# Exidekat/TransformerUpscaler

Measured on AMD Instinct MI355X. Metric: images/sec, FastTransformer 2x 720p->1080p inference, higher is better.
Workload: dtype bf16

## Files before the change

### transformerupscaler_amd/csrc/conv12_fused.hip

```cpp
#include "conv_pingpong.h"

namespace {

constexpr int TH = 8, TW = 32, HALO_W = TW + 2, HALO_H = TH + 2, NPIX_HALO = HALO_H * HALO_W;
constexpr int IN_BYTES = NPIX_HALO * 128;
constexpr int WROWS = 64, WSLAB = WROWS * 128;
constexpr int NRUNS = (NPIX_HALO + 15) / 16;
constexpr int RUNS_PER_WAVE = (NRUNS + 3) / 4;
constexpr size_t C12_LDS = (size_t)9 * WSLAB + 2 * (size_t)IN_BYTES + 256 + 256 + 256;
static_assert(C12_LDS <= 163840, "LDS budget");

__global__ __launch_bounds__(256) void conv1_compact_kernel(const float* __restrict__ x, u32x2* __restrict__ xc, int H, int W,
                                                            int Hp, int Wp)
{
    const int xp = blockIdx.y * 256 + threadIdx.x;
    if (xp >= Wp) return;
    const int row = blockIdx.x, b = row / Hp, yp = row - b * Hp;
    const int iy = yp - 2, ix = xp - 2;
    float v0 = 0.f, v1 = 0.f, v2 = 0.f;
    if (iy >= 0 && iy < H && ix >= 0 && ix < W) {
        const size_t plane = (size_t)H * W;
        const float* s = x + (size_t)b * 3 * plane + (size_t)iy * W + ix;
        v0 = s[0]; v1 = s[plane]; v2 = s[2 * plane];
    }
    xc[(size_t)row * Wp + xp] = u32x2{pack_bf16x2(v0, v1), pack_bf16x2(v2, 0.f)};
}

__global__ __launch_bounds__(512, 2) void conv12_fused_kernel(
    const bf16_t* __restrict__ xc, const bf16_t* __restrict__ w1, const float* __restrict__ b1,
    const bf16_t* __restrict__ wp, const float* __restrict__ bias, bf16_t* __restrict__ out,
    int B, int H, int W, int Wp, int img_bytes, int tilesX, int tilesY)
{
    extern __shared__ __attribute__((aligned(16))) char smem[];
    char* w_lds = smem;
    char* in_lds = smem + 9 * WSLAB;

    const int grp = __builtin_amdgcn_readfirstlane((int)(threadIdx.x >> 8));
    const int tid = threadIdx.x & 255, lane = tid & 63, wave = tid >> 6;
    const int wave_u = __builtin_amdgcn_readfirstlane(wave);
    const int g = lane >> 4, p = lane & 15;
    const int total_tiles = tilesX * tilesY * B;
    char* my_in = in_lds + grp * IN_BYTES;
    float* bias_lds = reinterpret_cast<float*>(in_lds + 2 * IN_BYTES);
    uint32_t* tab_lds = reinterpret_cast<uint32_t*>(in_lds + 2 * IN_BYTES + 512);

    uint32_t poff[9][2];
    pixel_frag_offsets<3, HALO_W>(poff, my_in, wave, g, p);
    const uint32_t wbase0 = weight_frag_base(w_lds, g, p);

    f32x4 acc[4][4];
    const uint32_t bias_addr = lds_addr(bias_lds) + (uint32_t)(g * 64);

    auto store_tile = [&](const TC& c) {
#pragma unroll
        for (int pg = 0; pg < 4; ++pg) {
            const int oy = c.ty * TH + 2 * wave + (pg >> 1);
            const int ox = c.tx * TW + (pg & 1) * 16 + p;
            const bool ok = oy < H && ox < W;
            const size_t eoff = (((size_t)c.b * H + oy) * W + ox) * 64 + g * 16;
            uint32_t pk[8];
#pragma unroll
            for (int ct = 0; ct < 4; ++ct) {
                pk[ct * 2 + 0] = relu_pack_bf16x2(acc[pg][ct][0], acc[pg][ct][1]);
                pk[ct * 2 + 1] = relu_pack_bf16x2(acc[pg][ct][2], acc[pg][ct][3]);
            }
            bf16_t* o = ok ? out + eoff : reinterpret_cast<bf16_t*>(tup_store_sink) + lane * 16;
            *reinterpret_cast<u32x4*>(o) = u32x4{pk[0], pk[1], pk[2], pk[3]};
            *reinterpret_cast<u32x4*>(o + 8) = u32x4{pk[4], pk[5], pk[6], pk[7]};
        }
    };

    struct Conv1In { uint32_t raw[RUNS_PER_WAVE][8]; bf16x8 a[4]; };
    auto issue_conv1_loads = [&](const TC& c, Conv1In& in) {
        const int l = lane_id_fresh(), lg = l >> 4, lp = l & 15;
        const bf16_t* wrow = w1 + lp * 32 + lg * 8;
#pragma unroll
        for (int ct = 0; ct < 4; ++ct) in.a[ct] = *reinterpret_cast<const bf16x8*>(wrow + ct * 512);
        const u32x4 so = *reinterpret_cast<const u32x4*>(tab_lds + lg * 16);
        const uint32_t so4 = tab_lds[lg * 16 + 4];
        const int cb = __builtin_amdgcn_readfirstlane(c.b), cty = __builtin_amdgcn_readfirstlane(c.ty);
        const int ctx = __builtin_amdgcn_readfirstlane(c.tx);
        const char* img = reinterpret_cast<const char*>(xc) + (size_t)cb * img_bytes;
        const __amdgpu_buffer_rsrc_t rs = __builtin_amdgcn_make_buffer_rsrc((void*)img, 0, img_bytes, 0x00020000);
        const int tbase = (cty * TH * Wp + ctx * TW) * 8;
#pragma unroll
        for (int j = 0; j < RUNS_PER_WAVE; ++j) {
            const int G = wave_u + 4 * j;
            const int q = min(16 * G + lp, NPIX_HALO - 1);
            const int hy = (q * 241) >> 13, hx = q - hy * HALO_W;
            const int pix = (hy * Wp + hx) * 8;
            uint32_t* r = in.raw[j];
            r[0] = __builtin_amdgcn_raw_buffer_load_b32(rs, pix + (int)so[0] + 4, tbase, 0);
            const u32x2 s1 = __builtin_amdgcn_raw_buffer_load_b64(rs, pix + (int)so[1], tbase, 0);
            const u32x2 s2 = __builtin_amdgcn_raw_buffer_load_b64(rs, pix + (int)so[2], tbase, 0);
            const u32x2 s3 = __builtin_amdgcn_raw_buffer_load_b64(rs, pix + (int)so[3], tbase, 0);
            r[7] = __builtin_amdgcn_raw_buffer_load_b32(rs, pix + (int)so4, tbase, 0);
            r[1] = s1[0]; r[2] = s1[1]; r[3] = s2[0]; r[4] = s2[1]; r[5] = s3[0]; r[6] = s3[1];
        }
    };
    auto build_conv1 = [&](const TC& c, const Conv1In& in) {
        const int l = lane_id_fresh(), lg = l >> 4, lp = l & 15;
        const u32x4 sel = *reinterpret_cast<const u32x4*>(tab_lds + lg * 16 + 8);
        f32x4 bv[4];
#pragma unroll
        for (int ct = 0; ct < 4; ++ct) bv[ct] = *reinterpret_cast<const f32x4*>(bias_lds + 64 + lg * 16 + ct * 4);
        const int ty0 = c.ty * TH, tx0 = c.tx * TW;
        const bool edge = !(ty0 >= 1 && ty0 + TH + 1 <= H && tx0 >= 1 && tx0 + TW + 1 <= W);
        const uint32_t img_lds = lds_addr(my_in);
#pragma unroll
        for (int j = 0; j < RUNS_PER_WAVE; ++j) {
            const int G = wave_u + 4 * j;
            const uint32_t* r = in.raw[j];
            const u32x4 bw = {__builtin_amdgcn_perm(r[1], r[0], sel[0]), __builtin_amdgcn_perm(r[3], r[2], sel[1]),
                              __builtin_amdgcn_perm(r[5], r[4], sel[2]), __builtin_amdgcn_perm(r[7], r[6], sel[3])};
            const bf16x8 bfrag = __builtin_bit_cast(bf16x8, bw);
            f32x4 a[4];
#pragma unroll
            for (int ct = 0; ct < 4; ++ct) a[ct] = mfma16x16x32(in.a[ct], bfrag, bv[ct]);
            uint32_t pk[8];
#pragma unroll
            for (int ct = 0; ct < 4; ++ct) {
                pk[ct * 2 + 0] = relu_pack_bf16x2(a[ct][0], a[ct][1]);
                pk[ct * 2 + 1] = relu_pack_bf16x2(a[ct][2], a[ct][3]);
            }
            const int q = 16 * G + lp;
            if (edge) {
                const int hy = (q * 241) >> 13, hx = q - hy * HALO_W;
                const bool ok = (unsigned)(ty0 - 1 + hy) < (unsigned)H && (unsigned)(tx0 - 1 + hx) < (unsigned)W;
#pragma unroll
                for (int k = 0; k < 8; ++k) pk[k] = ok ? pk[k] : 0u;
            }
            const uint32_t a0 = img_lds + (uint32_t)swz128(q, 2 * lg), a1 = a0 ^ 16u;
            if (q < NPIX_HALO) {
                *reinterpret_cast<__attribute__((address_space(3))) u32x4*>(a0) = u32x4{pk[0], pk[1], pk[2], pk[3]};
                *reinterpret_cast<__attribute__((address_space(3))) u32x4*>(a1) = u32x4{pk[4], pk[5], pk[6], pk[7]};
            }
            __builtin_amdgcn_sched_barrier(0);
        }
    };

    const TileWalk walk(total_tiles, tilesX, tilesY, grp, true);
    const int my_count = walk.my_count, nphases = walk.nphases;
    const TC c_first = walk.first;

    stage_weights<4, 9>(w_lds, wp);
    if (threadIdx.x < 128) bias_lds[threadIdx.x] = threadIdx.x < 64 ? bias[threadIdx.x] : b1[threadIdx.x - 64];
    if (threadIdx.x < 64) {
        constexpr uint32_t X = 0x05040100u, Y = 0x01000706u, Z = 0x07060504u, F = 0x03020100u, Zero = 0x0c0c0c0cu;
        constexpr int slot_dydx[4][5] = {{0x00, 0x00, 0x01, 0x01, 0x02}, {0x02, 0x10, 0x10, 0x11, 0x12},
                                         {0x12, 0x12, 0x20, 0x21, 0x21}, {0x22, 0x22, 0x22, 0x22, 0x22}};
        constexpr uint32_t sels[4][4] = {{Z, X, Y, Z}, {X, Y, Z, X}, {Y, Z, X, Y}, {Z, F, Zero, Zero}};
        const int gg = threadIdx.x >> 4, w = threadIdx.x & 15;
        uint32_t v = 0u;
        if (w < 5) v = (uint32_t)((((slot_dydx[gg][w] >> 4) * Wp) + (slot_dydx[gg][w] & 15)) * 8);
        else if (w >= 8 && w < 12) v = sels[gg][w - 8];
        tab_lds[threadIdx.x] = v;
    }
    __syncthreads();
    if (grp == 0 && my_count > 0) {
        Conv1In in;
        issue_conv1_loads(c_first, in);
        build_conv1(c_first, in);
    }
    asm volatile("s_waitcnt lgkmcnt(0)" ::: "memory");
    __syncthreads();
    TC c_done = c_first, c_next = c_first;
    if (grp == 0) walk.advance(c_next);

    for (int ph = 0; ph < nphases; ++ph) {
        const int k = ph >> 1;
        if ((ph & 1) == grp) {
            if (k < my_count) k_loop<4, 9>(acc, poff, wbase0, bias_addr);
        } else {
            const int done = grp == 0 ? k : k - 1;
            const int nxt = done + 1;
            const bool store = done >= 0 && done < my_count;
            const bool fetch = nxt < my_count;
            if (fetch && store) {
                Conv1In in;
                issue_conv1_loads(c_next, in);
                __builtin_amdgcn_sched_barrier(0);
                store_tile(c_done);
                __builtin_amdgcn_sched_barrier(0);
                build_conv1(c_next, in);
            } else if (fetch) {
                Conv1In in;
                issue_conv1_loads(c_next, in);
                build_conv1(c_next, in);
            } else if (store) {
                store_tile(c_done);
            }
            c_done = c_next;
            walk.advance(c_next);
        }
        asm volatile("s_waitcnt lgkmcnt(0)" ::: "memory");
        __builtin_amdgcn_s_barrier();
    }
    asm volatile("s_waitcnt vmcnt(0)" ::: "memory");
}

}

extern "C" int tup_conv1_compact_fwd(const float* x, void* xc, int B, int H, int W, void* stream)
{
    if (B <= 0 || H <= 0 || W <= 0) return 0;
    const int Hp = (H + TH - 1) / TH * TH + 4, Wp = (W + TW - 1) / TW * TW + 4;
    if ((long long)B * Hp > 0x7fffffffLL) return (int)hipErrorInvalidValue;
    conv1_compact_kernel<<<dim3((unsigned)(B * Hp), (unsigned)((Wp + 255) / 256)), dim3(256), 0, reinterpret_cast<hipStream_t>(stream)>>>(
        x, (u32x2*)xc, H, W, Hp, Wp);
    TUP_CHECK_LAUNCH();
    return 0;
}

extern "C" int tup_conv12_fused_fwd(const void* xc, const void* w1, const float* b1, const void* w2, const float* b2, void* out,
                                    int B, int H, int W, void* stream)
{
    if (B <= 0 || H <= 0 || W <= 0) return 0;
    const int tilesX = (W + TW - 1) / TW, tilesY = (H + TH - 1) / TH;
    const int Hp = tilesY * TH + 4, Wp = tilesX * TW + 4;
    const long long nt = (long long)tilesX * tilesY * B;
    if (nt > 0x7fffffffLL || (long long)Hp * Wp * 8 > 0x7fffffffLL) return (int)hipErrorInvalidValue;
    hipStream_t s = reinterpret_cast<hipStream_t>(stream);
    TUP_SET_DYN_LDS(conv12_fused_kernel, C12_LDS);
    const int grid = (int)(nt < 256 ? nt : 256);
    conv12_fused_kernel<<<dim3(grid), dim3(512), C12_LDS, s>>>((const bf16_t*)xc, (const bf16_t*)w1, b1, (const bf16_t*)w2, b2,
                                                               (bf16_t*)out, B, H, W, Wp, Hp * Wp * 8, tilesX, tilesY);
    TUP_CHECK_LAUNCH();
    return 0;
}
```

### transformerupscaler_amd/csrc/conv_pingpong.h

```cpp
#pragma once
#include "common.h"

namespace {

[[maybe_unused]] __device__ __attribute__((aligned(16))) unsigned int tup_zero_line[4] = {0u, 0u, 0u, 0u};
[[maybe_unused]] __device__ __attribute__((aligned(16))) unsigned int tup_store_sink[64 * 8];

#define TUP_ADD_DPP(acc, v, ctrl) asm("v_add_f32_dpp %0, %1, %0 " ctrl " row_mask:0xf bank_mask:0xf bound_ctrl:1" : "+v"(acc) : "v"(v))

TUP_DEVICE uint32_t relu_pack_bf16x2(float lo, float hi) {
    typedef short s16x2 __attribute__((ext_vector_type(2)));
    const bf16x2 v = __builtin_convertvector(f32x2{lo, hi}, bf16x2);
    return __builtin_bit_cast(uint32_t, __builtin_elementwise_max(__builtin_bit_cast(s16x2, v), s16x2{0, 0}));
}

TUP_DEVICE void xcd_band(int total, bool use_bands, int& first, int& stride, int& limit) {
    if ((gridDim.x & 7) == 0 && use_bands) {
        const int band = (total + 7) >> 3, start = (blockIdx.x & 7) * band;
        limit = min(total, start + band);
        first = start + (blockIdx.x >> 3);
        stride = gridDim.x >> 3;
    } else {
        limit = total; first = blockIdx.x; stride = gridDim.x;
    }
}

struct TC { int tx, ty, b; };

struct TileWalk {
    int my_count;
    int nphases;
    TC first;
    int tilesX, tilesY, step_x, step_y, step_b;

    TUP_DEVICE TileWalk(int total_tiles, int tilesX_, int tilesY_, int grp, bool use_bands) : tilesX(tilesX_), tilesY(tilesY_) {
        int first0, per, limit;
        xcd_band(total_tiles, use_bands, first0, per, limit);
        const int first_tile = first0 + grp * per, stride = 2 * per;
        my_count = first_tile < limit ? (limit - first_tile + stride - 1) / stride : 0;
        const int cnt0 = first0 < limit ? (limit - first0 + stride - 1) / stride : 0;
        nphases = 2 * cnt0 + 1;
        first.tx = first_tile % tilesX; const int t = first_tile / tilesX; first.ty = t % tilesY; first.b = t / tilesY;
        step_x = stride % tilesX; step_y = (stride / tilesX) % tilesY; step_b = stride / (tilesX * tilesY);
    }
    TUP_DEVICE void advance(TC& c) const {
        c.tx += step_x;
        if (c.tx >= tilesX) { c.tx -= tilesX; ++c.ty; }
        c.ty += step_y; c.b += step_b;
        if (c.ty >= tilesY) { c.ty -= tilesY; ++c.b; }
    }
};

template <int HALO_H, int HALO_W, int PAD>
struct HaloDma {
    static constexpr int IN_CHUNKS = HALO_H * HALO_W * 8, NPIECE = (IN_CHUNKS + 255) / 256;
    static constexpr bool LAST_PARTIAL = (IN_CHUNKS % 256) != 0;
    int rel[NPIECE];
    int tid, wave;
    bool last_ok;

    TUP_DEVICE HaloDma(int W, int tid_) : tid(tid_), wave(tid_ >> 6), last_ok((NPIECE - 1) * 256 + tid_ < IN_CHUNKS) {
#pragma unroll
        for (int it = 0; it < NPIECE; ++it) {
            const int idx = LAST_PARTIAL ? min(it * 256 + tid, IN_CHUNKS - 1) : it * 256 + tid;
            const int q = idx >> 3, c = (idx & 7) ^ ((q >> 1) & 7);
            const int yy = q / HALO_W, xx = q - yy * HALO_W;
            rel[it] = ((yy - PAD) * W + (xx - PAD)) * 128 + c * 16;
        }
    }
    TUP_DEVICE void prefetch(const bf16_t* x, int b, int ty0, int tx0, int H, int W, char* my_in, const void* zero) const {
        const char* xb = reinterpret_cast<const char*>(x + (size_t)b * H * W * 64);
        if (ty0 >= PAD && ty0 + HALO_H - PAD <= H && tx0 >= PAD && tx0 + HALO_W - PAD <= W) {
            const char* tb = xb + ((size_t)ty0 * W + tx0) * 128;
#pragma unroll
            for (int it = 0; it < NPIECE; ++it) {
                if (LAST_PARTIAL && it == NPIECE - 1 && !last_ok) continue;
                __builtin_amdgcn_global_load_lds((const __attribute__((address_space(1))) void*)(tb + rel[it]),
                                                 (__attribute__((address_space(3))) void*)(my_in + (it * 256 + wave * 64) * 16), 16, 0, 0);
            }
            return;
        }
#pragma unroll 1
        for (int base = 0; base < IN_CHUNKS; base += 256) {
            const int idx = base + tid;
            if (!LAST_PARTIAL || idx < IN_CHUNKS) {
                const int q = idx >> 3, cphys = idx & 7;
                const int c = cphys ^ ((q >> 1) & 7);
                const int yy = q / HALO_W, xx = q - yy * HALO_W;
                const int iy = ty0 - PAD + yy, ix = tx0 - PAD + xx;
                const void* src = (iy >= 0 && iy < H && ix >= 0 && ix < W)
                                      ? (const void*)(xb + ((size_t)(iy * W + ix) * 128 + c * 16)) : zero;
                __builtin_amdgcn_global_load_lds((const __attribute__((address_space(1))) void*)src,
                                                 (__attribute__((address_space(3))) void*)(my_in + (base + wave * 64) * 16), 16, 0, 0);
            }
        }
    }
};

template <int KS, int HALO_W>
TUP_DEVICE void pixel_frag_offsets(uint32_t (&poff)[KS * KS][2], const char* my_in, int wave, int g, int p) {
#pragma unroll
    for (int tap = 0; tap < KS * KS; ++tap)
#pragma unroll
        for (int rw = 0; rw < 2; ++rw)
            poff[tap][rw] = lds_addr(my_in) + (uint32_t)swz128((2 * wave + rw) * HALO_W + p + (tap / KS) * HALO_W + (tap % KS), g);
}
TUP_DEVICE uint32_t weight_frag_base(const char* w_lds, int g, int p) { return lds_addr(w_lds) + (uint32_t)swz128(p, g); }

template <int CT, int NTAPS>
TUP_DEVICE void k_loop(f32x4 (&acc)[4][CT], const uint32_t (&poff)[NTAPS][2], uint32_t wbase0, uint32_t bias_addr) {
    constexpr int WROWS = CT * 16;
    const uint32_t wbase1 = wbase0 ^ 64u;
    const uint32_t wbase0h = wbase0 + 57344u, wbase1h = wbase1 + 57344u;
#pragma unroll
    for (int ct = 0; ct < CT; ++ct) acc[0][ct] = __builtin_bit_cast(f32x4, lds_read_b128_asm(bias_addr + ct * 16));
    lds_wait<0>();
#pragma unroll
    for (int pg = 1; pg < 4; ++pg)
#pragma unroll
        for (int ct = 0; ct < CT; ++ct) acc[pg][ct] = acc[0][ct];
    constexpr int NSTEPS = NTAPS * 2;
    constexpr int PER = 4 + CT;
    constexpr int NM = 4 * CT;
    bf16x8 pf[3][4], wf[3][CT];
    auto load_one = [&](int step, int slot, int j) {
        const int tap = step >> 1;
        if (j < 4) {
            pf[slot][j] = (step & 1) ? lds_read_b128_asm_off_x64(poff[tap][j >> 1], (j & 1) * 2048)
                                     : lds_read_b128_asm_off(poff[tap][j >> 1], (j & 1) * 2048);
        } else {
            const int ct = j - 4;
            const int woff = (tap * WROWS + ct * 16) * 128;
            wf[slot][ct] = woff < 57344 ? lds_read_b128_asm_off((step & 1) ? wbase1 : wbase0, woff)
                                        : lds_read_b128_asm_off((step & 1) ? wbase1h : wbase0h, woff - 57344);
        }
    };
#pragma unroll
    for (int j = 0; j < PER; ++j) load_one(0, 0, j);
#pragma unroll
    for (int j = 0; j < PER; ++j) load_one(1, 1, j);
#pragma unroll
    for (int step = 0; step < NSTEPS; ++step) {
        const int cur = step % 3;
        if (step + 1 < NSTEPS) lds_wait<PER>(); else lds_wait<0>();
        __builtin_amdgcn_sched_barrier(0);
        int rd = 0;
#pragma unroll
        for (int m = 0; m < NM; ++m) {
            if (step + 2 < NSTEPS) {
#pragma unroll
                for (int j = 0; j < PER; ++j)
                    if (j == rd && j * NM < (m + 1) * PER) { load_one(step + 2, (step + 2) % 3, j); ++rd; }
            }
            const int pg = m / CT, ct = m % CT;
            acc[pg][ct] = mfma16x16x32(wf[cur][ct], pf[cur][pg], acc[pg][ct]);
            __builtin_amdgcn_sched_barrier(0);
        }
    }
}

template <int CT, int NTAPS>
TUP_DEVICE void stage_weights(char* w_lds, const bf16_t* wsrc) {
    for (int idx = threadIdx.x; idx < NTAPS * CT * 16 * 8; idx += 512) {
        const int row = idx >> 3, c = idx & 7;
        *reinterpret_cast<u32x4*>(w_lds + swz128(row, c)) = *reinterpret_cast<const u32x4*>(wsrc + (size_t)idx * 8);
    }
}
template <int CT, bool THIN>
TUP_DEVICE void stage_bias(float* bias_lds, const float* bias, int nt, int cout_valid) {
    if (threadIdx.x < 16 * CT) {
        const int gg = threadIdx.x / (4 * CT), ct = (threadIdx.x / 4) % CT, e = threadIdx.x & 3;
        float bval = 0.f;
        if (bias) {
            if constexpr (!THIN) bval = bias[nt * 64 + gg * 16 + ct * 4 + e];
            else { const int co = 16 * ct + 4 * gg + e; bval = co < cout_valid ? bias[co] : 0.f; }
        }
        bias_lds[threadIdx.x] = bval;
    }
}

}
```

### transformerupscaler_amd/csrc/decoder_fused.hip

```cpp
#include "conv_pingpong.h"

namespace {

constexpr int TH = 8, TW = 32, HALO_W = TW + 2, HALO_H = TH + 2, NPIX_HALO = HALO_H * HALO_W;
constexpr int IN_BYTES = NPIX_HALO * 128;
constexpr int WROWS = 64, WSLAB = WROWS * 128;
constexpr size_t DEC_LDS = (size_t)9 * WSLAB + 2 * (size_t)IN_BYTES + 256;
static_assert(DEC_LDS <= 163840, "LDS budget");

__global__ __launch_bounds__(512, 2) void decoder_fused_kernel(
    const bf16_t* __restrict__ x, const bf16_t* __restrict__ wp, const float* __restrict__ bias,
    const bf16_t* __restrict__ wz, float* __restrict__ part, float* __restrict__ seamv, float* __restrict__ cseam,
    int B, int H, int W, int tilesX, int tilesY)
{
    extern __shared__ __attribute__((aligned(16))) char smem[];
    char* w_lds = smem;
    char* in_lds = smem + 9 * WSLAB;

    const int grp = __builtin_amdgcn_readfirstlane((int)(threadIdx.x >> 8));
    const int tid = threadIdx.x & 255, lane = tid & 63, wave = tid >> 6;
    const int g = lane >> 4, p = lane & 15;
    const int total_tiles = tilesX * tilesY * B;
    char* my_in = in_lds + grp * IN_BYTES;

    using Dma = HaloDma<HALO_H, HALO_W, 1>;
    constexpr int NPIECE = Dma::NPIECE;
    const Dma dma(W, tid);
    auto prefetch_tile = [&](const TC& c) { dma.prefetch(x, c.b, c.ty * TH, c.tx * TW, H, W, my_in, tup_zero_line); };

    uint32_t poff[9][2];
    pixel_frag_offsets<3, HALO_W>(poff, my_in, wave, g, p);
    const uint32_t wbase0 = weight_frag_base(w_lds, g, p);

    f32x4 acc[4][4];
    float* bias_lds = reinterpret_cast<float*>(in_lds + 2 * IN_BYTES);
    const uint32_t bias_addr = lds_addr(bias_lds) + (uint32_t)(g * 64);
    bf16x8 zf[3][2];
    const uint32_t wz_voff = (uint32_t)(p * 128 + g * 16);
    auto load_zf = [&]() {
#pragma unroll
        for (int dy = 0; dy < 3; ++dy) {
            const bf16_t* base = wz + dy * 1024;
            asm volatile("global_load_dwordx4 %0, %1, %2" : "=v"(zf[dy][0]) : "v"(wz_voff), "s"(base));
            asm volatile("global_load_dwordx4 %0, %1, %2 offset:64" : "=v"(zf[dy][1]) : "v"(wz_voff), "s"(base));
        }
    };

    auto store_tile = [&](const TC& c) {
        const int b = c.b, y0 = c.ty * TH + 2 * wave, x0 = c.tx * TW;
        const bool edge = c.ty * TH + TH > H || x0 + TW > W;
        f32x4 z[4][3];
#pragma unroll
        for (int pg = 0; pg < 4; ++pg) {
            typedef short s16x2 __attribute__((ext_vector_type(2)));
            uint32_t pk[8];
#pragma unroll
            for (int ct = 0; ct < 4; ++ct) {
                pk[ct * 2 + 0] = pack_bf16x2(acc[pg][ct][0], acc[pg][ct][1]);
                pk[ct * 2 + 1] = pack_bf16x2(acc[pg][ct][2], acc[pg][ct][3]);
            }
#pragma unroll
            for (int q = 0; q < 8; ++q)
                pk[q] = __builtin_bit_cast(uint32_t, __builtin_elementwise_max(__builtin_bit_cast(s16x2, pk[q]), s16x2{0, 0}));
            if (edge) {
                const bool ok = y0 + (pg >> 1) < H && x0 + (pg & 1) * 16 + p < W;
#pragma unroll
                for (int q = 0; q < 8; ++q) pk[q] = ok ? pk[q] : 0u;
            }
            const bf16x8 b0 = __builtin_bit_cast(bf16x8, u32x4{pk[0], pk[1], pk[2], pk[3]});
            const bf16x8 b1 = __builtin_bit_cast(bf16x8, u32x4{pk[4], pk[5], pk[6], pk[7]});
#pragma unroll
            for (int dy = 0; dy < 3; ++dy) {
                z[pg][dy] = mfma16x16x32(zf[dy][0], b0, f32x4{0.f, 0.f, 0.f, 0.f});
                z[pg][dy] = mfma16x16x32(zf[dy][1], b1, z[pg][dy]);
            }
        }
        __builtin_amdgcn_sched_barrier(0);
        asm volatile("s_nop 7\n\ts_nop 7\n\ts_nop 4" ::: "memory");
        __builtin_amdgcn_sched_barrier(0);
        float h[2][2][3];
#pragma unroll
        for (int rw = 0; rw < 2; ++rw)
#pragma unroll
            for (int dy = 0; dy < 3; ++dy) {
                const f32x4 l = z[2 * rw][dy], r = z[2 * rw + 1][dy];
                float v0 = l[1], v1 = r[1];
                TUP_ADD_DPP(v0, l[0], "row_shr:1"); TUP_ADD_DPP(v0, l[2], "row_shl:1"); TUP_ADD_DPP(v0, r[2], "row_shr:15");
                TUP_ADD_DPP(v1, r[0], "row_shr:1"); TUP_ADD_DPP(v1, r[2], "row_shl:1"); TUP_ADD_DPP(v1, l[0], "row_shl:15");
                h[rw][0][dy] = v0; h[rw][1][dy] = v1;
            }
        const bool live = g < 3;
        const int plane = H * W, nrec = 3 * plane * 4;
        const __amdgpu_buffer_rsrc_t rp = __builtin_amdgcn_make_buffer_rsrc(part + (size_t)b * 3 * plane, 0, nrec, 0x00020000);
        const __amdgpu_buffer_rsrc_t rs = __builtin_amdgcn_make_buffer_rsrc(seamv + (size_t)b * 3 * plane, 0, nrec, 0x00020000);
        const int crec = H * tilesX * 128;
        const __amdgpu_buffer_rsrc_t rc = __builtin_amdgcn_make_buffer_rsrc(cseam + (size_t)b * H * tilesX * 32, 0, crec, 0x00020000);
        const int cbase = (g * plane + y0 * W) * 4;
#pragma unroll
        for (int cg = 0; cg < 2; ++cg) {
            const int ox = x0 + cg * 16 + p;
            const bool colok = live && ox < W;
            const int o = cbase + ox * 4, rowb = W * 4;
            const float o0 = h[0][cg][1] + h[1][cg][2], o1 = h[0][cg][0] + h[1][cg][1];
            __builtin_amdgcn_raw_buffer_store_b32(__builtin_bit_cast(uint32_t, o0), rp, colok && y0 < H ? o : nrec, 0, 0);
            __builtin_amdgcn_raw_buffer_store_b32(__builtin_bit_cast(uint32_t, o1), rp, colok && y0 + 1 < H ? o + rowb : nrec, 0, 0);
            __builtin_amdgcn_raw_buffer_store_b32(__builtin_bit_cast(uint32_t, h[0][cg][2]), rs,
                                                  colok && y0 >= 1 && y0 < H ? o - rowb : nrec, 0, 0);
            __builtin_amdgcn_raw_buffer_store_b32(__builtin_bit_cast(uint32_t, h[1][cg][0]), rs,
                                                  colok && y0 + 2 < H ? o + 2 * rowb : nrec, 0, 0);
        }
#pragma unroll
        for (int rw = 0; rw < 2; ++rw) {
            const int y = y0 + rw;
            const bool left = p == 0;
            const f32x4 v = left ? f32x4{z[2 * rw][0][2], z[2 * rw][1][2], z[2 * rw][2][2], 0.f}
                                 : f32x4{z[2 * rw + 1][0][0], z[2 * rw + 1][1][0], z[2 * rw + 1][2][0], 0.f};
            const bool ok = live & (y < H) & (left | ((p == 15) & (x0 + TW <= W)));
            const int off = ((y * tilesX + c.tx) * 2 + (left ? 0 : 1)) * 64 + g * 16;
            __builtin_amdgcn_raw_buffer_store_b128(__builtin_bit_cast(u32x4, v), rc, ok ? off : crec, 0, 0);
        }
    };
    constexpr int NSTORES = 10;

    const TileWalk walk(total_tiles, tilesX, tilesY, grp, true);
    const int my_count = walk.my_count, nphases = walk.nphases;
    const TC c_first = walk.first;

    stage_weights<4, 9>(w_lds, wp);
    stage_bias<4, false>(bias_lds, bias, 0, 64);
    if (grp == 0 && my_count > 0) prefetch_tile(c_first);
    __syncthreads();
    TC c_done = c_first, c_next = c_first;
    if (grp == 0) walk.advance(c_next);

    for (int ph = 0; ph < nphases; ++ph) {
        const int k = ph >> 1;
        if ((ph & 1) == grp) {
            if (k < my_count) k_loop<4, 9>(acc, poff, wbase0, bias_addr);
        } else {
            const int done = grp == 0 ? k : k - 1;
            const int nxt = done + 1;
            const bool store = done >= 0 && done < my_count;
            const bool fetch = nxt < my_count;
            if (store) load_zf();
            if (fetch) prefetch_tile(c_next);
            if (store) {
                if (fetch) asm volatile("s_waitcnt vmcnt(%0)" ::"n"(NPIECE - 1) : "memory");
                else asm volatile("s_waitcnt vmcnt(0)" ::: "memory");
                store_tile(c_done);
                asm volatile("s_waitcnt vmcnt(%0)" ::"n"(NSTORES) : "memory");
            } else {
                asm volatile("s_waitcnt vmcnt(0)" ::: "memory");
            }
            c_done = c_next;
            walk.advance(c_next);
        }
        asm volatile("s_waitcnt lgkmcnt(0)" ::: "memory");
        __builtin_amdgcn_s_barrier();
    }
    asm volatile("s_waitcnt vmcnt(0)" ::: "memory");
}

template <int V>
__global__ __launch_bounds__(256) void decoder_finish_kernel(
    float* __restrict__ res, const float* __restrict__ seamv, const float* __restrict__ cseam, const float* __restrict__ bias,
    int H, int W, int tilesX)
{
    typedef float fv __attribute__((ext_vector_type(V)));
    const int x0 = (blockIdx.x * 256 + threadIdx.x) * V;
    if (x0 >= W) return;
    const int row = blockIdx.y, b = row / H, y = row - b * H;
    const size_t plane = (size_t)H * W;
    const int ys = (y & 1) ? y + 1 : y - 1;
    const bool has_seam = ys >= 0 && ys < H;
    const size_t o0 = (size_t)b * 3 * plane + (size_t)y * W + x0;
#pragma unroll
    for (int c = 0; c < 3; ++c) {
        const size_t o = o0 + c * plane;
        fv v = *reinterpret_cast<const fv*>(res + o);
        const fv sv = has_seam ? *reinterpret_cast<const fv*>(seamv + o) : fv{};
#pragma unroll
        for (int e = 0; e < V; ++e) {
            const int xq = x0 + e;
            float t = bias[c] + v[e];
            if (has_seam) t += sv[e];
            int ctile = -1, side = 0;
            if ((xq & 31) == 31 && xq + 1 < W) { ctile = (xq >> 5) + 1; side = 0; }
            else if ((xq & 31) == 0 && xq > 0) { ctile = (xq >> 5) - 1; side = 1; }
            if (ctile >= 0) {
#pragma unroll
                for (int dy = 0; dy < 3; ++dy) {
                    const int yy = y + dy - 1;
                    if (yy >= 0 && yy < H) t += cseam[((((size_t)b * H + yy) * tilesX + ctile) * 2 + side) * 16 + c * 4 + dy];
                }
            }
            v[e] = t;
        }
        *reinterpret_cast<fv*>(res + o) = v;
    }
}

}

namespace {
int launch_decoder_parts(const void* x, const void* w1, const float* b1, const void* wz, float* part, float* seamv, float* cseam,
                         int B, int H, int W, void* stream)
{
    const int tilesX = (W + TW - 1) / TW, tilesY = (H + TH - 1) / TH;
    const long long nt = (long long)tilesX * tilesY * B;
    if (nt > 0x7fffffffLL || (long long)H * W * 12 > 0x7fffffffLL || (long long)H * tilesX * 128 > 0x7fffffffLL)
        return (int)hipErrorInvalidValue;
    hipStream_t s = reinterpret_cast<hipStream_t>(stream);
    TUP_SET_DYN_LDS(decoder_fused_kernel, DEC_LDS);
    const int grid = (int)(nt < 256 ? nt : 256);
    decoder_fused_kernel<<<dim3(grid), dim3(512), DEC_LDS, s>>>((const bf16_t*)x, (const bf16_t*)w1, b1, (const bf16_t*)wz, part,
                                                                 seamv, cseam, B, H, W, tilesX, tilesY);
    TUP_CHECK_LAUNCH();
    return 0;
}
}

extern "C" int tup_decoder_fused_fwd(const void* x, const void* w1, const float* b1, const void* wz, const float* b2,
                                     float* seamv, float* cseam, float* out, int B, int H, int W, void* stream)
{
    if (B <= 0 || H <= 0 || W <= 0) return 0;
    const int tilesX = (W + TW - 1) / TW;
    if (const int err = launch_decoder_parts(x, w1, b1, wz, out, seamv, cseam, B, H, W, stream)) return err;
    hipStream_t s = reinterpret_cast<hipStream_t>(stream);
    if ((long long)B * H > 0x7fffffffLL) return (int)hipErrorInvalidValue;
    if (W % 4 == 0)
        decoder_finish_kernel<4><<<dim3((unsigned)((W / 4 + 255) / 256), (unsigned)(B * H)), dim3(256), 0, s>>>(out, seamv, cseam, b2, H, W, tilesX);
    else
        decoder_finish_kernel<1><<<dim3((unsigned)((W + 255) / 256), (unsigned)(B * H)), dim3(256), 0, s>>>(out, seamv, cseam, b2, H, W, tilesX);
    TUP_CHECK_LAUNCH();
    return 0;
}

extern "C" int tup_decoder_fused_parts_fwd(const void* x, const void* w1, const float* b1, const void* wz,
                                           float* part, float* seamv, float* cseam, int B, int H, int W, void* stream)
{
    if (B <= 0 || H <= 0 || W <= 0) return 0;
    return launch_decoder_parts(x, w1, b1, wz, part, seamv, cseam, B, H, W, stream);
}
```

Before: 2740.

## Trim address math in conv12/decoder stores and loads, raise producer wave priority

Replaces per-pixel 64-bit address computation and sink-pointer stores with buffer-resource stores that use row-based offsets and out-of-range clamping. Precomputes halo pixel offsets into an LDS table so the conv1 load loop skips the divide-by-multiply math, and uses a single base LDS address with constant strides for the conv1 writes. Raises wave priority (s_setprio) for the load/store group during ping-pong phases. Also adds optional diagnostic phase timestamps that compile away without TUP_DIAG. The aim is fewer VALU/SALU instructions on the memory side, at the cost of a small extra LDS table and more complex bounds handling.

```diff
diff --git a/transformerupscaler_amd/csrc/conv12_fused.hip b/transformerupscaler_amd/csrc/conv12_fused.hip
--- a/transformerupscaler_amd/csrc/conv12_fused.hip
+++ b/transformerupscaler_amd/csrc/conv12_fused.hip
@@ -7,8 +7,10 @@
 constexpr int WROWS = 64, WSLAB = WROWS * 128;
 constexpr int NRUNS = (NPIX_HALO + 15) / 16;
 constexpr int RUNS_PER_WAVE = (NRUNS + 3) / 4;
-constexpr size_t C12_LDS = (size_t)9 * WSLAB + 2 * (size_t)IN_BYTES + 256 + 256 + 256;
+constexpr size_t C12_LDS = (size_t)9 * WSLAB + 2 * (size_t)IN_BYTES + 256 + 256 + 256 + 2048;
+static_assert(16 * (3 + 4 * (RUNS_PER_WAVE - 2)) + 15 < NPIX_HALO, "every run but a wave's last lies inside the halo image");
 static_assert(C12_LDS <= 163840, "LDS budget");
+TUP_PHASE_STAMPS_DECL(tup_conv12_stamps);
 
 __global__ __launch_bounds__(256) void conv1_compact_kernel(const float* __restrict__ x, u32x2* __restrict__ xc, int H, int W,
                                                             int Hp, int Wp)
@@ -43,6 +45,7 @@
     char* my_in = in_lds + grp * IN_BYTES;
     float* bias_lds = reinterpret_cast<float*>(in_lds + 2 * IN_BYTES);
     uint32_t* tab_lds = reinterpret_cast<uint32_t*>(in_lds + 2 * IN_BYTES + 512);
+    uint32_t* pix_lds = tab_lds + 64;
 
     uint32_t poff[9][2];
     pixel_frag_offsets<3, HALO_W>(poff, my_in, wave, g, p);
@@ -52,21 +55,27 @@
     const uint32_t bias_addr = lds_addr(bias_lds) + (uint32_t)(g * 64);
 
     auto store_tile = [&](const TC& c) {
-#pragma unroll
-        for (int pg = 0; pg < 4; ++pg) {
-            const int oy = c.ty * TH + 2 * wave + (pg >> 1);
-            const int ox = c.tx * TW + (pg & 1) * 16 + p;
-            const bool ok = oy < H && ox < W;
-            const size_t eoff = (((size_t)c.b * H + oy) * W + ox) * 64 + g * 16;
-            uint32_t pk[8];
-#pragma unroll
-            for (int ct = 0; ct < 4; ++ct) {
-                pk[ct * 2 + 0] = relu_pack_bf16x2(acc[pg][ct][0], acc[pg][ct][1]);
-                pk[ct * 2 + 1] = relu_pack_bf16x2(acc[pg][ct][2], acc[pg][ct][3]);
-            }
-            bf16_t* o = ok ? out + eoff : reinterpret_cast<bf16_t*>(tup_store_sink) + lane * 16;
-            *reinterpret_cast<u32x4*>(o) = u32x4{pk[0], pk[1], pk[2], pk[3]};
-            *reinterpret_cast<u32x4*>(o + 8) = u32x4{pk[4], pk[5], pk[6], pk[7]};
+        const int oy0 = c.ty * TH + 2 * wave_u, x0 = c.tx * TW;
+        const int rowbytes = W * 128;
+        const int lane_o = (x0 + p) * 128 + g * 32;
+#pragma unroll
+        for (int rw = 0; rw < 2; ++rw) {
+            const bool rok = oy0 + rw < H;
+            bf16_t* const rowp = out + ((size_t)c.b * H + (rok ? oy0 + rw : 0)) * W * 64;
+            const __amdgpu_buffer_rsrc_t rr = __builtin_amdgcn_make_buffer_rsrc(rowp, 0, rok ? rowbytes : 0, 0x00020000);
+#pragma unroll
+            for (int cg = 0; cg < 2; ++cg) {
+                const int pg = 2 * rw + cg;
+                const int o = x0 + cg * 16 + p < W ? lane_o + cg * 2048 : rowbytes;
+                uint32_t pk[8];
+#pragma unroll
+                for (int ct = 0; ct < 4; ++ct) {
+                    pk[ct * 2 + 0] = relu_pack_bf16x2(acc[pg][ct][0], acc[pg][ct][1]);
+                    pk[ct * 2 + 1] = relu_pack_bf16x2(acc[pg][ct][2], acc[pg][ct][3]);
+                }
+                __builtin_amdgcn_raw_buffer_store_b128(u32x4{pk[0], pk[1], pk[2], pk[3]}, rr, o, 0, 0);
+                __builtin_amdgcn_raw_buffer_store_b128(u32x4{pk[4], pk[5], pk[6], pk[7]}, rr, o + 16, 0, 0);
+            }
         }
     };
 
@@ -78,6 +87,10 @@
         for (int ct = 0; ct < 4; ++ct) in.a[ct] = *reinterpret_cast<const bf16x8*>(wrow + ct * 512);
         const u32x4 so = *reinterpret_cast<const u32x4*>(tab_lds + lg * 16);
         const uint32_t so4 = tab_lds[lg * 16 + 4];
+        const uint32_t* pt = pix_lds + (wave_u * 16 + lp) * 8;
+        const u32x4 px03 = *reinterpret_cast<const u32x4*>(pt);
+        const u32x2 px45 = *reinterpret_cast<const u32x2*>(pt + 4);
+        const int pixj[RUNS_PER_WAVE] = {(int)px03[0], (int)px03[1], (int)px03[2], (int)px03[3], (int)px45[0], (int)px45[1]};
         const int cb = __builtin_amdgcn_readfirstlane(c.b), cty = __builtin_amdgcn_readfirstlane(c.ty);
         const int ctx = __builtin_amdgcn_readfirstlane(c.tx);
         const char* img = reinterpret_cast<const char*>(xc) + (size_t)cb * img_bytes;
@@ -85,10 +98,7 @@
         const int tbase = (cty * TH * Wp + ctx * TW) * 8;
 #pragma unroll
         for (int j = 0; j < RUNS_PER_WAVE; ++j) {
-            const int G = wave_u + 4 * j;
-            const int q = min(16 * G + lp, NPIX_HALO - 1);
-            const int hy = (q * 241) >> 13, hx = q - hy * HALO_W;
-            const int pix = (hy * Wp + hx) * 8;
+            const int pix = pixj[j];
             uint32_t* r = in.raw[j];
             r[0] = __builtin_amdgcn_raw_buffer_load_b32(rs, pix + (int)so[0] + 4, tbase, 0);
             const u32x2 s1 = __builtin_amdgcn_raw_buffer_load_b64(rs, pix + (int)so[1], tbase, 0);
@@ -106,7 +116,10 @@
         for (int ct = 0; ct < 4; ++ct) bv[ct] = *reinterpret_cast<const f32x4*>(bias_lds + 64 + lg * 16 + ct * 4);
         const int ty0 = c.ty * TH, tx0 = c.tx * TW;
         const bool edge = !(ty0 >= 1 && ty0 + TH + 1 <= H && tx0 >= 1 && tx0 + TW + 1 <= W);
-        const uint32_t img_lds = lds_addr(my_in);
+        typedef __attribute__((address_space(3))) char lds_char;
+        const uint32_t a0 = lds_addr(my_in) + (uint32_t)swz128(16 * wave_u + lp, 2 * lg);
+        lds_char* const w0 = reinterpret_cast<lds_char*>(a0);
+        lds_char* const w1 = reinterpret_cast<lds_char*>(a0 ^ 16u);
 #pragma unroll
         for (int j = 0; j < RUNS_PER_WAVE; ++j) {
             const int G = wave_u + 4 * j;
@@ -123,17 +136,16 @@
                 pk[ct * 2 + 0] = relu_pack_bf16x2(a[ct][0], a[ct][1]);
                 pk[ct * 2 + 1] = relu_pack_bf16x2(a[ct][2], a[ct][3]);
             }
-            const int q = 16 * G + lp;
             if (edge) {
+                const int q = 16 * G + lp;
                 const int hy = (q * 241) >> 13, hx = q - hy * HALO_W;
                 const bool ok = (unsigned)(ty0 - 1 + hy) < (unsigned)H && (unsigned)(tx0 - 1 + hx) < (unsigned)W;
 #pragma unroll
                 for (int k = 0; k < 8; ++k) pk[k] = ok ? pk[k] : 0u;
             }
-            const uint32_t a0 = img_lds + (uint32_t)swz128(q, 2 * lg), a1 = a0 ^ 16u;
-            if (q < NPIX_HALO) {
-                *reinterpret_cast<__attribute__((address_space(3))) u32x4*>(a0) = u32x4{pk[0], pk[1], pk[2], pk[3]};
-                *reinterpret_cast<__attribute__((address_space(3))) u32x4*>(a1) = u32x4{pk[4], pk[5], pk[6], pk[7]};
+            if (j < RUNS_PER_WAVE - 1 || 16 * G + lp < NPIX_HALO) {
+                *reinterpret_cast<__attribute__((address_space(3))) u32x4*>(w0 + j * 8192) = u32x4{pk[0], pk[1], pk[2], pk[3]};
+                *reinterpret_cast<__attribute__((address_space(3))) u32x4*>(w1 + j * 8192) = u32x4{pk[4], pk[5], pk[6], pk[7]};
             }
             __builtin_amdgcn_sched_barrier(0);
         }
@@ -156,6 +168,12 @@
         else if (w >= 8 && w < 12) v = sels[gg][w - 8];
         tab_lds[threadIdx.x] = v;
     }
+    {
+        const int w = threadIdx.x >> 7, pp = (threadIdx.x >> 3) & 15, j = threadIdx.x & 7;
+        const int q = min(16 * (w + 4 * j) + pp, NPIX_HALO - 1);
+        const int hy = q / HALO_W, hx = q - hy * HALO_W;
+        pix_lds[threadIdx.x] = j < RUNS_PER_WAVE ? (uint32_t)((hy * Wp + hx) * 8) : 0u;
+    }
     __syncthreads();
     if (grp == 0 && my_count > 0) {
         Conv1In in;
@@ -167,11 +185,15 @@
     TC c_done = c_first, c_next = c_first;
     if (grp == 0) walk.advance(c_next);
 
+    TUP_PHASE_STAMPS_BEGIN(tup_conv12_stamps);
     for (int ph = 0; ph < nphases; ++ph) {
         const int k = ph >> 1;
+        TUP_PHASE_STAMP(0);
         if ((ph & 1) == grp) {
             if (k < my_count) k_loop<4, 9>(acc, poff, wbase0, bias_addr);
+            TUP_PHASE_STAMP(1);
         } else {
+            __builtin_amdgcn_s_setprio(2);
             const int done = grp == 0 ? k : k - 1;
             const int nxt = done + 1;
             const bool store = done >= 0 && done < my_count;
@@ -182,19 +204,26 @@
                 __builtin_amdgcn_sched_barrier(0);
                 store_tile(c_done);
                 __builtin_amdgcn_sched_barrier(0);
+                TUP_PHASE_STAMP(1);
                 build_conv1(c_next, in);
             } else if (fetch) {
                 Conv1In in;
                 issue_conv1_loads(c_next, in);
+                TUP_PHASE_STAMP(1);
                 build_conv1(c_next, in);
             } else if (store) {
                 store_tile(c_done);
+                TUP_PHASE_STAMP(1);
             }
             c_done = c_next;
             walk.advance(c_next);
+            __builtin_amdgcn_s_setprio(0);
         }
         asm volatile("s_waitcnt lgkmcnt(0)" ::: "memory");
+        TUP_PHASE_STAMP(2);
         __builtin_amdgcn_s_barrier();
+        TUP_PHASE_STAMP(3);
+        TUP_PHASE_STAMPS_STORE(tup_conv12_stamps, grp, ph);
     }
     asm volatile("s_waitcnt vmcnt(0)" ::: "memory");
 }
@@ -219,12 +248,20 @@
     const int tilesX = (W + TW - 1) / TW, tilesY = (H + TH - 1) / TH;
     const int Hp = tilesY * TH + 4, Wp = tilesX * TW + 4;
     const long long nt = (long long)tilesX * tilesY * B;
-    if (nt > 0x7fffffffLL || (long long)Hp * Wp * 8 > 0x7fffffffLL) return (int)hipErrorInvalidValue;
+    if (nt > 0x7fffffffLL || (long long)Hp * Wp * 8 > 0x7fffffffLL || (long long)W * 128 > 0x7fffffffLL) return (int)hipErrorInvalidValue;
     hipStream_t s = reinterpret_cast<hipStream_t>(stream);
     TUP_SET_DYN_LDS(conv12_fused_kernel, C12_LDS);
+    TUP_PHASE_STAMPS_ARM(tup_conv12_stamps);
     const int grid = (int)(nt < 256 ? nt : 256);
     conv12_fused_kernel<<<dim3(grid), dim3(512), C12_LDS, s>>>((const bf16_t*)xc, (const bf16_t*)w1, b1, (const bf16_t*)w2, b2,
                                                                (bf16_t*)out, B, H, W, Wp, Hp * Wp * 8, tilesX, tilesY);
     TUP_CHECK_LAUNCH();
     return 0;
 }
+
+#ifdef TUP_DIAG
+extern "C" int tup_debug_conv12_stamps(unsigned long long* host_out)
+{
+    return (int)hipMemcpyFromSymbol(host_out, HIP_SYMBOL(tup_conv12_stamps), sizeof(unsigned long long) * 2 * 16 * 4);
+}
+#endif
diff --git a/transformerupscaler_amd/csrc/conv_pingpong.h b/transformerupscaler_amd/csrc/conv_pingpong.h
--- a/transformerupscaler_amd/csrc/conv_pingpong.h
+++ b/transformerupscaler_amd/csrc/conv_pingpong.h
@@ -13,6 +13,25 @@
     const bf16x2 v = __builtin_convertvector(f32x2{lo, hi}, bf16x2);
     return __builtin_bit_cast(uint32_t, __builtin_elementwise_max(__builtin_bit_cast(s16x2, v), s16x2{0, 0}));
 }
+
+#ifdef TUP_DIAG
+#define TUP_PHASE_STAMPS_DECL(sym) __device__ unsigned long long sym[2][16][4]; __device__ int sym##_on
+#define TUP_PHASE_STAMPS_BEGIN(sym) \
+    const bool st_on_ = sym##_on && blockIdx.x == 100 && (threadIdx.x & 255) == 0; \
+    unsigned long long st_[4] = {0, 0, 0, 0}
+#define TUP_PHASE_STAMP(i) do { __builtin_amdgcn_sched_barrier(0); \
+        asm volatile("s_memtime %0\n\ts_waitcnt lgkmcnt(0)" : "=s"(st_[i]) :: "memory"); __builtin_amdgcn_sched_barrier(0); } while (0)
+#define TUP_PHASE_STAMPS_STORE(sym, grp, ph) do { if (st_on_ && (ph) < 16) { \
+        sym[grp][ph][0] = st_[0]; sym[grp][ph][1] = st_[1]; sym[grp][ph][2] = st_[2]; sym[grp][ph][3] = st_[3]; } } while (0)
+#define TUP_PHASE_STAMPS_ARM(sym) do { const int on_ = TUP_ENV_FLAG("TUP_CONV_STAMPS") ? 1 : 0; \
+        hipError_t e_ = hipMemcpyToSymbol(HIP_SYMBOL(sym##_on), &on_, sizeof(int)); if (e_ != hipSuccess) return (int)e_; } while (0)
+#else
+#define TUP_PHASE_STAMPS_DECL(sym)
+#define TUP_PHASE_STAMPS_BEGIN(sym) do {} while (0)
+#define TUP_PHASE_STAMP(i) do {} while (0)
+#define TUP_PHASE_STAMPS_STORE(sym, grp, ph) do {} while (0)
+#define TUP_PHASE_STAMPS_ARM(sym) do {} while (0)
+#endif
 
 TUP_DEVICE void xcd_band(int total, bool use_bands, int& first, int& stride, int& limit) {
     if ((gridDim.x & 7) == 0 && use_bands) {
diff --git a/transformerupscaler_amd/csrc/decoder_fused.hip b/transformerupscaler_amd/csrc/decoder_fused.hip
--- a/transformerupscaler_amd/csrc/decoder_fused.hip
+++ b/transformerupscaler_amd/csrc/decoder_fused.hip
@@ -7,6 +7,7 @@
 constexpr int WROWS = 64, WSLAB = WROWS * 128;
 constexpr size_t DEC_LDS = (size_t)9 * WSLAB + 2 * (size_t)IN_BYTES + 256;
 static_assert(DEC_LDS <= 163840, "LDS budget");
+TUP_PHASE_STAMPS_DECL(tup_decoder_stamps);
 
 __global__ __launch_bounds__(512, 2) void decoder_fused_kernel(
     const bf16_t* __restrict__ x, const bf16_t* __restrict__ wp, const float* __restrict__ bias,
@@ -46,22 +47,19 @@
         }
     };
 
+    const int wave_u = __builtin_amdgcn_readfirstlane(wave);
     auto store_tile = [&](const TC& c) {
-        const int b = c.b, y0 = c.ty * TH + 2 * wave, x0 = c.tx * TW;
+        const int b = c.b, y0 = c.ty * TH + 2 * wave_u, x0 = c.tx * TW;
         const bool edge = c.ty * TH + TH > H || x0 + TW > W;
         f32x4 z[4][3];
 #pragma unroll
         for (int pg = 0; pg < 4; ++pg) {
-            typedef short s16x2 __attribute__((ext_vector_type(2)));
             uint32_t pk[8];
 #pragma unroll
             for (int ct = 0; ct < 4; ++ct) {
-                pk[ct * 2 + 0] = pack_bf16x2(acc[pg][ct][0], acc[pg][ct][1]);
-                pk[ct * 2 + 1] = pack_bf16x2(acc[pg][ct][2], acc[pg][ct][3]);
-            }
-#pragma unroll
-            for (int q = 0; q < 8; ++q)
-                pk[q] = __builtin_bit_cast(uint32_t, __builtin_elementwise_max(__builtin_bit_cast(s16x2, pk[q]), s16x2{0, 0}));
+                pk[ct * 2 + 0] = relu_pack_bf16x2(acc[pg][ct][0], acc[pg][ct][1]);
+                pk[ct * 2 + 1] = relu_pack_bf16x2(acc[pg][ct][2], acc[pg][ct][3]);
+            }
             if (edge) {
                 const bool ok = y0 + (pg >> 1) < H && x0 + (pg & 1) * 16 + p < W;
 #pragma unroll
@@ -90,34 +88,39 @@
                 h[rw][0][dy] = v0; h[rw][1][dy] = v1;
             }
         const bool live = g < 3;
-        const int plane = H * W, nrec = 3 * plane * 4;
-        const __amdgpu_buffer_rsrc_t rp = __builtin_amdgcn_make_buffer_rsrc(part + (size_t)b * 3 * plane, 0, nrec, 0x00020000);
-        const __amdgpu_buffer_rsrc_t rs = __builtin_amdgcn_make_buffer_rsrc(seamv + (size_t)b * 3 * plane, 0, nrec, 0x00020000);
+        const int plane = H * W, nrec = 3 * plane * 4, rowb = W * 4;
+        float* const pimg = part + (size_t)b * 3 * plane;
+        float* const simg = seamv + (size_t)b * 3 * plane;
         const int crec = H * tilesX * 128;
-        const __amdgpu_buffer_rsrc_t rc = __builtin_amdgcn_make_buffer_rsrc(cseam + (size_t)b * H * tilesX * 32, 0, crec, 0x00020000);
-        const int cbase = (g * plane + y0 * W) * 4;
+        float* const cimg = cseam + (size_t)b * H * tilesX * 32;
+        const int lane_o = (g * plane + x0 + p) * 4;
+        const bool rok0 = y0 < H, rok1 = y0 + 1 < H, rokm = y0 >= 1 && y0 < H, rok2 = y0 + 2 < H;
+        const __amdgpu_buffer_rsrc_t rp0 = __builtin_amdgcn_make_buffer_rsrc(pimg, 0, rok0 ? nrec : 0, 0x00020000);
+        const __amdgpu_buffer_rsrc_t rp1 = __builtin_amdgcn_make_buffer_rsrc(pimg, 0, rok1 ? nrec : 0, 0x00020000);
+        const __amdgpu_buffer_rsrc_t rsm = __builtin_amdgcn_make_buffer_rsrc(simg, 0, rokm ? nrec : 0, 0x00020000);
+        const __amdgpu_buffer_rsrc_t rs2 = __builtin_amdgcn_make_buffer_rsrc(simg, 0, rok2 ? nrec : 0, 0x00020000);
+        const int so0 = rok0 ? y0 * rowb : 0, so1 = rok1 ? (y0 + 1) * rowb : 0;
+        const int som = rokm ? (y0 - 1) * rowb : 0, so2 = rok2 ? (y0 + 2) * rowb : 0;
 #pragma unroll
         for (int cg = 0; cg < 2; ++cg) {
-            const int ox = x0 + cg * 16 + p;
-            const bool colok = live && ox < W;
-            const int o = cbase + ox * 4, rowb = W * 4;
+            const int o = live && x0 + cg * 16 + p < W ? lane_o + cg * 64 : nrec;
             const float o0 = h[0][cg][1] + h[1][cg][2], o1 = h[0][cg][0] + h[1][cg][1];
-            __builtin_amdgcn_raw_buffer_store_b32(__builtin_bit_cast(uint32_t, o0), rp, colok && y0 < H ? o : nrec, 0, 0);
-            __builtin_amdgcn_raw_buffer_store_b32(__builtin_bit_cast(uint32_t, o1), rp, colok && y0 + 1 < H ? o + rowb : nrec, 0, 0);
-            __builtin_amdgcn_raw_buffer_store_b32(__builtin_bit_cast(uint32_t, h[0][cg][2]), rs,
-                                                  colok && y0 >= 1 && y0 < H ? o - rowb : nrec, 0, 0);
-            __builtin_amdgcn_raw_buffer_store_b32(__builtin_bit_cast(uint32_t, h[1][cg][0]), rs,
-                                                  colok && y0 + 2 < H ? o + 2 * rowb : nrec, 0, 0);
-        }
+            __builtin_amdgcn_raw_buffer_store_b32(__builtin_bit_cast(uint32_t, o0), rp0, o, so0, 0);
+            __builtin_amdgcn_raw_buffer_store_b32(__builtin_bit_cast(uint32_t, o1), rp1, o, so1, 0);
+            __builtin_amdgcn_raw_buffer_store_b32(__builtin_bit_cast(uint32_t, h[0][cg][2]), rsm, o, som, 0);
+            __builtin_amdgcn_raw_buffer_store_b32(__builtin_bit_cast(uint32_t, h[1][cg][0]), rs2, o, so2, 0);
+        }
+        const bool left = p == 0;
+        const bool cok = live & (left | ((p == 15) & (x0 + TW <= W)));
+        const int co = cok ? (left ? 0 : 64) + g * 16 : crec;
 #pragma unroll
         for (int rw = 0; rw < 2; ++rw) {
             const int y = y0 + rw;
-            const bool left = p == 0;
+            const bool rok = rw ? rok1 : rok0;
             const f32x4 v = left ? f32x4{z[2 * rw][0][2], z[2 * rw][1][2], z[2 * rw][2][2], 0.f}
                                  : f32x4{z[2 * rw + 1][0][0], z[2 * rw + 1][1][0], z[2 * rw + 1][2][0], 0.f};
-            const bool ok = live & (y < H) & (left | ((p == 15) & (x0 + TW <= W)));
-            const int off = ((y * tilesX + c.tx) * 2 + (left ? 0 : 1)) * 64 + g * 16;
-            __builtin_amdgcn_raw_buffer_store_b128(__builtin_bit_cast(u32x4, v), rc, ok ? off : crec, 0, 0);
+            const __amdgpu_buffer_rsrc_t rc = __builtin_amdgcn_make_buffer_rsrc(cimg, 0, rok ? crec : 0, 0x00020000);
+            __builtin_amdgcn_raw_buffer_store_b128(__builtin_bit_cast(u32x4, v), rc, co, rok ? (y * tilesX + c.tx) * 128 : 0, 0);
         }
     };
     constexpr int NSTORES = 10;
@@ -133,11 +136,15 @@
     TC c_done = c_first, c_next = c_first;
     if (grp == 0) walk.advance(c_next);
 
+    TUP_PHASE_STAMPS_BEGIN(tup_decoder_stamps);
     for (int ph = 0; ph < nphases; ++ph) {
         const int k = ph >> 1;
+        TUP_PHASE_STAMP(0);
         if ((ph & 1) == grp) {
             if (k < my_count) k_loop<4, 9>(acc, poff, wbase0, bias_addr);
+            TUP_PHASE_STAMP(1);
         } else {
+            __builtin_amdgcn_s_setprio(2);
             const int done = grp == 0 ? k : k - 1;
             const int nxt = done + 1;
             const bool store = done >= 0 && done < my_count;
@@ -148,15 +155,21 @@
                 if (fetch) asm volatile("s_waitcnt vmcnt(%0)" ::"n"(NPIECE - 1) : "memory");
                 else asm volatile("s_waitcnt vmcnt(0)" ::: "memory");
                 store_tile(c_done);
+                TUP_PHASE_STAMP(1);
                 asm volatile("s_waitcnt vmcnt(%0)" ::"n"(NSTORES) : "memory");
             } else {
+                TUP_PHASE_STAMP(1);
                 asm volatile("s_waitcnt vmcnt(0)" ::: "memory");
             }
             c_done = c_next;
             walk.advance(c_next);
+            __builtin_amdgcn_s_setprio(0);
         }
         asm volatile("s_waitcnt lgkmcnt(0)" ::: "memory");
+        TUP_PHASE_STAMP(2);
         __builtin_amdgcn_s_barrier();
+        TUP_PHASE_STAMP(3);
+        TUP_PHASE_STAMPS_STORE(tup_decoder_stamps, grp, ph);
     }
     asm volatile("s_waitcnt vmcnt(0)" ::: "memory");
 }
@@ -212,6 +225,7 @@
         return (int)hipErrorInvalidValue;
     hipStream_t s = reinterpret_cast<hipStream_t>(stream);
     TUP_SET_DYN_LDS(decoder_fused_kernel, DEC_LDS);
+    TUP_PHASE_STAMPS_ARM(tup_decoder_stamps);
     const int grid = (int)(nt < 256 ? nt : 256);
     decoder_fused_kernel<<<dim3(grid), dim3(512), DEC_LDS, s>>>((const bf16_t*)x, (const bf16_t*)w1, b1, (const bf16_t*)wz, part,
                                                                  seamv, cseam, B, H, W, tilesX, tilesY);
@@ -242,3 +256,10 @@
     if (B <= 0 || H <= 0 || W <= 0) return 0;
     return launch_decoder_parts(x, w1, b1, wz, part, seamv, cseam, B, H, W, stream);
 }
+
+#ifdef TUP_DIAG
+extern "C" int tup_debug_decoder_stamps(unsigned long long* host_out)
+{
+    return (int)hipMemcpyFromSymbol(host_out, HIP_SYMBOL(tup_decoder_stamps), sizeof(unsigned long long) * 2 * 16 * 4);
+}
+#endif
```

Result: no change. 2767, median of 6 (+1.0%).
